# febrianrachmadi/dep-gan-im

Hardware: AMD Instinct MI355X
Metric: 2D slices/sec (G+2D+GP train step), 256x256x1 fp32 (higher is better)
Workload: dtype f32; 1 GPU; DEP-GAN-IM twoCritics canonical train step (critic-Y2 + critic-DEM + G update, WGAN-GP), batch 32 per GPU, 256x256x1; per_gpu_batch=32, global_batch=32, parallelism=dp1

## Files before the change

### dep_gan_im_amd/csrc/common.h

```cpp
#pragma once
#include <hip/hip_runtime.h>
#include <stdint.h>
#include <stddef.h>

typedef float f32x2 __attribute__((ext_vector_type(2)));
typedef float f32x4 __attribute__((ext_vector_type(4)));
typedef float f32x16 __attribute__((ext_vector_type(16)));

struct TView {
  float* p;
  long sB, sY, sX;
};

static inline TView make_view(float* p, int H, int W, int C) {
  TView v;
  v.p = p;
  v.sX = C;
  v.sY = (long)W * C;
  v.sB = (long)H * W * C;
  return v;
}
static inline TView make_view_slice(float* p, int H, int W, int Ctot, int c0) {
  TView v = make_view(p, H, W, Ctot);
  v.p = p + c0;
// ... 28 lines not shown
  TViewH v;
  v.p = nullptr;
  v.sB = v.sY = v.sX = 0;
  return v;
}

struct Epilogue {
  const float* bias;
  const float* scale;
  const float* shift;
  const float* film_mul;
  const float* film_add;
  int film_ld;
  TView out_pre;
  TView res;
  TView mask;
  int relu;
  int accumulate;
  TView pool;
  const float* head_w;
  const float* head_b;
  float* head_out;
  int head_tanh, head_skip_out;
};

struct ConvArgs {
  TView in;
  TView out;
  const float* w;
  int B, H, W, Cin, Cout;
  Epilogue ep;
  long wsT, wsI, wsO;
  int flip;
  int vec4;
  unsigned long long* dbg;
  int groups;
  int lgx, lgy;
  const float* w_group[4];
  long out_group_off[4];
  int cpt;
  long in_run_off[4];
};

struct WgradArgs {
  TView x;
  TView dy;
  float* part;
  int B, H, W, Cin, Cout;
  int nTiles, tilesPerChunk;
  float* colpart;
  int colB;
};

#ifdef __HIPCC__
static __device__ __forceinline__ float dg_vmax(float a, float b) {
  float o;
  asm("v_max_f32 %0, %1, %2" : "=v"(o) : "v"(a), "v"(b));
  return o;
}
#endif

#define DG_OK 0
#define DG_ERR_ARG 1
#define DG_ERR_HIP 2
#define DG_ERR_UNSUPPORTED 3

void dg_set_error(const char* fmt, ...);
// ... 85 lines not shown
  const float* src;
  float* dst;
  const float* kscale;
  int ntaps, srcI, srcO, io, transpose, flip;
  int NT, CK, nCC, Kdim, Ndim;
  int bf16;
  int tapg;
  int wino;
  unsigned total;
  unsigned per_nt;
  unsigned nt_stride;
  unsigned blk0, nblk;
};
int dg_pack_job(const ConvPlan& pl, const float* src, int srcI, int srcO, int io, int transpose, int flip,
                const float* kscale, float* dst, size_t nt_stride, PackJob* job);
unsigned dg_pack_layout(PackJob* jobs_host, int njobs);
int dg_pack_weights_batch(const PackJob* jobs_dev, int njobs, unsigned nblocks, hipStream_t st);

int dg_pack_weights(const ConvPlan& pl, const float* src, int srcI, int srcO, int io, int transpose, int flip,
                    const float* kscale, float* dst, hipStream_t st);

int dg_conv_igemm(const ConvPlan& pl, const ConvArgs& a, hipStream_t st);
int dg_conv_igemm_check(const ConvPlan& pl, const ConvArgs& a);
bool dg_conv_igemm_wp_supported(const ConvPlan& pl, const ConvArgs& a, bool force);
int dg_conv_igemm_wp(const ConvPlan& pl, const ConvArgs& a, hipStream_t st);
bool dg_conv_igemm_ws5_supported(const ConvPlan& pl, const ConvArgs& a, bool force);
int dg_conv_igemm_ws5(const ConvPlan& pl, const ConvArgs& a, hipStream_t st);
const char* dg_conv_igemm_ws5_name(const ConvPlan& pl);
int dg_conv_igemm_tile(const ConvPlan& pl, const ConvArgs& a, hipStream_t st);
bool dg_conv_igemm_head_supported(const ConvPlan& pl, const ConvArgs& a);
ConvPlan dg_plan_conv_wino(int Cin, int Cout);
bool dg_conv_wino_supported(const ConvPlan& pl, const ConvArgs& a);
const char* dg_conv_wino_name(const ConvArgs& a);
int dg_conv_wino(const ConvPlan& pl, const ConvArgs& a, hipStream_t st);
enum { DG_EPF_BIAS = 1, DG_EPF_AFFINE = 2, DG_EPF_FILM = 4, DG_EPF_RELU = 8, DG_EPF_PRE = 16, DG_EPF_RES = 32,
       DG_EPF_MASK = 64, DG_EPF_POOL = 128, DG_EPF_ACCUM = 256, DG_EPF_HEAD = 512, DG_EPF_ALL = 1023 };
unsigned dg_epilogue_flags(const Epilogue& e);
int dg_wino_epi_class(unsigned flags, int form);
void dg_set_epi_classes(int on);
int dg_get_epi_classes();
void dg_conv_igemm_name(const ConvPlan& pl, const ConvArgs& a, char* buf, size_t cap);
int dg_conv_direct(int KS, const ConvArgs& a, hipStream_t st);

int dg_wgrad(int KS, const WgradArgs& a, int* nchunks, hipStream_t st);
int dg_wgrad_finish(const float* part, int nchunks, int ntaps, int Cin, int Cout, const float* scale, float* out,
                    float* raw, int accumulate, int oi, const float* colpart, int colC, const float* colscale,
                    float* colout, float* colraw, hipStream_t st);
int dg_wgrad_finish_rows(const float* part, int nchunks, int ntaps, int Cin, int Cout, const float* scale, float* out,
                         float* raw, int accumulate, int oi, const float* colpart, int colrows, int colC,
                         const float* colscale, float* colout, float* colraw, hipStream_t st);

bool dg_wgrad_bf16_supported(int KS, int Cin, int Cout);
int dg_wgrad_bf16(int KS, const WgradArgs& a, int* nchunks, hipStream_t st);

int dg_wgrad_small(int KS, const WgradArgs& a, int* nchunks, hipStream_t st);

int dg_wgrad_plan(int KS, int B, int H, int W, int Cin, int Cout, int out[4]);
int dg_wgrad_small_plan(int KS, int B, int H, int W, int Cin, int Cout, int out[4]);
int dg_wgrad_bf16_plan(int KS, int B, int H, int W, int Cin, int Cout, int out[4]);

enum DgWgradKernel { DG_WG_F32 = 0, DG_WG_EDGE = 1, DG_WG_BF16 = 2, DG_WG_BF16S = 3, DG_WG_DECONV = 4 };
struct DgWgradChoice {
  int kernel, nchunks;
  size_t part_floats;
  int col_rows;
};
// ... 3 lines not shown
```

### dep_gan_im_amd/csrc/igemm_epilogue.inc

```
#ifndef EPI_PRE_SYNC
#define EPI_PRE_SYNC __syncthreads()
#define EPI_PRE_SYNC_DEFAULTED
#endif
  EPI_PRE_SYNC;
  constexpr int CP = NT + 4;
#ifdef EPI_ES_BASE
  float* es = EPI_ES_BASE;
#else
  float* es = smem + wv * (64 * CP);
#endif
  constexpr int NQ = (MF == 32) ? 4 : 1, CSTEP = (MF == 32) ? 8 : 4;
#if defined(EPI_STAGE)
  EPI_STAGE;
  (void)es;
#elif !defined(EPI_PHASED)
#pragma unroll
  for (int mt = 0; mt < MT; ++mt)
#pragma unroll
    for (int g = 0; g < NQ; ++g) {
      f32x4 q4;
#pragma unroll
      for (int k = 0; k < 4; ++k) q4[k] = acc[mt][4 * g + k];
      *reinterpret_cast<f32x4*>(es + (MF * mt + r) * CP + CSTEP * g + 4 * h) = q4;
    }
// ... 10 lines not shown
#ifndef EPI_OYW
  const int wvu = __builtin_amdgcn_readfirstlane(wv);
#endif
  const Epilogue& e = a.ep;
#ifdef EPI_CLASS
  typedef EPI_CLASS EpiC;
  constexpr bool EPI_CT = EpiC::fixed;
  const bool affine = EPI_CT ? EpiC::affine : (e.scale != nullptr), film = EPI_CT ? EpiC::film : (e.film_mul != nullptr),
             relu = EPI_CT ? EpiC::relu : (e.relu != 0), accum = EPI_CT ? false : (e.accumulate != 0);
  const bool has_bias = EPI_CT ? EpiC::bias : (e.bias != nullptr), has_pre = EPI_CT ? EpiC::pre : (e.out_pre.p != nullptr),
             has_res = EPI_CT ? EpiC::res : (e.res.p != nullptr), has_msk = EPI_CT ? EpiC::msk : (e.mask.p != nullptr),
             has_pool = EPI_CT ? EpiC::pool : (e.pool.p != nullptr);
#else
  const bool affine = e.scale != nullptr, film = e.film_mul != nullptr, relu = e.relu != 0, accum = e.accumulate != 0;
  const bool has_bias = e.bias != nullptr, has_pre = e.out_pre.p != nullptr, has_res = e.res.p != nullptr,
             has_msk = e.mask.p != nullptr, has_pool = e.pool.p != nullptr;
#endif
#ifdef EPI_OYW
  const int oyw = EPI_OYW;
#else
  const int oyw = ty0 + 4 * wvu;
#endif
#ifdef EPI_HEAD
  float hkeep_out = 0.f;
#endif
#ifdef EPI_FULL
  const bool full = EPI_FULL;
#else
  const bool full = (ty0 + 16 <= a.H) && (tx0 + 16 <= a.W);
#endif
  if (co < a.Cout) {
    f32x4 bias4 = {0.f, 0.f, 0.f, 0.f}, sc4 = {1.f, 1.f, 1.f, 1.f}, sh4 = {0.f, 0.f, 0.f, 0.f};
    f32x4 fm4 = {1.f, 1.f, 1.f, 1.f}, fa4 = {0.f, 0.f, 0.f, 0.f};
    if (has_bias) bias4 = *reinterpret_cast<const f32x4*>(e.bias + co);
    if (affine) {
      sc4 = *reinterpret_cast<const f32x4*>(e.scale + co);
      sh4 = *reinterpret_cast<const f32x4*>(e.shift + co);
    }
#pragma unroll
    for (int k = 0; k < 4; ++k) sh4[k] = fmaf(bias4[k], sc4[k], sh4[k]);
    if (film) {
      fm4 = *reinterpret_cast<const f32x4*>(e.film_mul + (long)b * e.film_ld + co);
      fa4 = *reinterpret_cast<const f32x4*>(e.film_add + (long)b * e.film_ld + co);
    }
    auto mk = [&](const float* p) {
      const unsigned long long u = (unsigned long long)p;
      const unsigned lo = __builtin_amdgcn_readfirstlane((unsigned)u), hi = __builtin_amdgcn_readfirstlane((unsigned)(u >> 32));
      return __builtin_amdgcn_make_buffer_rsrc((void*)(((unsigned long long)hi << 32) | lo), 0, 0x7FFFFFFF, 0x00020000);
    };
    const int lo_out = 4 * (pl0 * (int)a.out.sX + co);
    const int lo_pre = has_pre ? 4 * (pl0 * (int)e.out_pre.sX + co) : 0;
    const int lo_res = has_res ? 4 * (pl0 * (int)e.res.sX + co) : 0;
    const int lo_msk = has_msk ? 4 * (pl0 * (int)e.mask.sX + co) : 0;
    const __amdgpu_buffer_rsrc_t r_out = mk(a.out.p + out_goff + view_off(a.out, b, oyw, tx0));
    const __amdgpu_buffer_rsrc_t r_pre = mk(has_pre ? e.out_pre.p + view_off(e.out_pre, b, oyw, tx0) : a.out.p);
    const __amdgpu_buffer_rsrc_t r_res = mk(has_res ? e.res.p + view_off(e.res, b, oyw, tx0) : a.out.p);
    const __amdgpu_buffer_rsrc_t r_msk = mk(has_msk ? e.mask.p + view_off(e.mask, b, oyw, tx0) : a.out.p);
    const __amdgpu_buffer_rsrc_t r_pool =
        mk(has_pool ? e.pool.p + view_off(e.pool, b, oyw >> 1, tx0 >> 1) : a.out.p);
    const int lo_pool = has_pool ? 4 * ((pl0 >> 1) * (int)e.pool.sX + co) : 0;
    const int sY_pool = 4 * (int)e.pool.sY, sX_pool = 4 * (int)e.pool.sX;
    f32x4 vrow = {0.f, 0.f, 0.f, 0.f};
#ifdef EPI_HEAD
#ifdef EPI_CLASS
    const bool has_head = EPI_HEAD && (EPI_CT ? EpiC::head : (e.head_out != nullptr));
#else
    const bool has_head = EPI_HEAD && e.head_out != nullptr;
#endif
    f32x4 hw4 = {0.f, 0.f, 0.f, 0.f};
    if (has_head) hw4 = *reinterpret_cast<const f32x4*>(e.head_w + co);
    const bool skip_out = has_head && e.head_skip_out != 0;
#else
    constexpr bool has_head = false, skip_out = false;
#endif
    typedef int i32x4 __attribute__((ext_vector_type(4)));
    auto ld = [&](const __amdgpu_buffer_rsrc_t& r, int voff, int soff) {
      const i32x4 t = __builtin_amdgcn_raw_buffer_load_b128(r, voff, soff, 0);
      return __builtin_bit_cast(f32x4, t);
    };
    auto st = [&](const __amdgpu_buffer_rsrc_t& r, int voff, int soff, f32x4 v) {
      __builtin_amdgcn_raw_buffer_store_b128(__builtin_bit_cast(i32x4, v), r, voff, soff, 0);
    };
    const int sY_out = 4 * (int)a.out.sY, sX_out = 4 * (int)a.out.sX;
    const int sY_pre = 4 * (int)e.out_pre.sY, sX_pre = 4 * (int)e.out_pre.sX;
    const int sY_res = 4 * (int)e.res.sY, sX_res = 4 * (int)e.res.sX;
    const int sY_msk = 4 * (int)e.mask.sY, sX_msk = 4 * (int)e.mask.sX;
#ifdef EPI_STAGE_LATE
    EPI_STAGE_LATE;
#endif
#pragma unroll
    for (int p = 0; p < NPASS; ++p) {
      constexpr int RP = 16 / PPP;
      const int py = (p & 1) + 2 * (p / (2 * RP)), px0 = ((p >> 1) % RP) * PPP;
      const bool ok = full || (oyw + py < a.H && tx0 + px0 + pl0 < a.W);
#if defined(EPI_FETCH)
      f32x4 v;
      EPI_FETCH(v, py, (px0 + pl0));
#elif defined(EPI_PHASED)
      static_assert(MF == 32, "phased epilogue: 32-pixel tiles");
      if (p % (NPASS / MT) == 0) {
        const int mtp = p / (NPASS / MT);
#pragma unroll
        for (int g = 0; g < NQ; ++g) {
          f32x4 q4;
#pragma unroll
          for (int k = 0; k < 4; ++k) q4[k] = acc[mtp][4 * g + k];
          *reinterpret_cast<f32x4*>(es + r * CP + CSTEP * g + 4 * h) = q4;
        }
      }
      f32x4 v = *reinterpret_cast<const f32x4*>(es + ((py & 1) * 16 + px0 + pl0) * CP + c4);
#else
      f32x4 v = *reinterpret_cast<const f32x4*>(es + (py * 16 + px0 + pl0) * CP + c4);
#endif
#pragma unroll
      for (int k = 0; k < 4; ++k) v[k] = fmaf(v[k], sc4[k], sh4[k]);
      if (has_pre) {
        if (ok) st(r_pre, lo_pre, py * sY_pre + px0 * sX_pre, v);
      }
      if (film) {
#pragma unroll
        for (int k = 0; k < 4; ++k) v[k] = film_preact(v[k], fm4[k], fa4[k]);
      }
      if (relu) {
#pragma unroll
        for (int k = 0; k < 4; ++k) v[k] = dg_vmax(v[k], 0.f);
      }
      if (has_res) {
        f32x4 rr = {0.f, 0.f, 0.f, 0.f};
        if (ok) rr = ld(r_res, lo_res, py * sY_res + px0 * sX_res);
#pragma unroll
        for (int k = 0; k < 4; ++k) v[k] += rr[k];
      }
      if (has_msk) {
        f32x4 mm = {1.f, 1.f, 1.f, 1.f};
        if (ok) mm = ld(r_msk, lo_msk, py * sY_msk + px0 * sX_msk);
#pragma unroll
        for (int k = 0; k < 4; ++k) v[k] = (mm[k] > 0.f) ? v[k] : 0.f;
      }
      const int so = py * sY_out + px0 * sX_out;
      if (accum) {
        f32x4 old = {0.f, 0.f, 0.f, 0.f};
        if (ok) old = ld(r_out, lo_out, so);
#pragma unroll
        for (int k = 0; k < 4; ++k) v[k] += old[k];
      }
      if (ok && !skip_out) st(r_out, lo_out, so, v);
#ifdef EPI_HEAD
      if (has_head) {
        static_assert(!EPI_HEAD || (NT == 32 && NPASS == 8), "fused head: 32-channel tiles, eight passes");
        float d = v[0] * hw4[0];
        d = fmaf(v[1], hw4[1], d);
        d = fmaf(v[2], hw4[2], d);
        d = fmaf(v[3], hw4[3], d);
#define EPI_DPP(x, ctrl) \
  __builtin_bit_cast(float, __builtin_amdgcn_update_dpp(0, __builtin_bit_cast(int, (x)), (ctrl), 0xF, 0xF, false))
        d += EPI_DPP(d, 0xB1);
        d += EPI_DPP(d, 0x4E);
        d += EPI_DPP(d, 0x141);
#undef EPI_DPP
        hkeep_out = ((lane & 7) == p) ? d : hkeep_out;
      }
#endif
      if (has_pool) {
        if ((py & 1) == 0) {
          vrow = v;
        } else {
          f32x4 m;
#pragma unroll
          for (int k = 0; k < 4; ++k) {
            const float t = dg_vmax(vrow[k], v[k]);
            m[k] = dg_vmax(t, __shfl_xor(t, LPP, 64));
          }
          if (ok && (pl0 & 1) == 0) st(r_pool, lo_pool, (py >> 1) * sY_pool + (px0 >> 1) * sX_pool, m);
        }
      }
    }
  }
#ifdef EPI_HEAD
  if (EPI_HEAD && a.ep.head_out != nullptr && n0 < a.Cout) {
    const int ph = lane & 7, plh = lane >> 3;
    const int pyh = (ph & 1) + 2 * (ph >> 2), pxh = ((ph >> 1) & 1) * 8 + plh;
    const int yh = oyw + pyh, xh = tx0 + pxh;
    if (yh < a.H && xh < a.W) {
      const float t = hkeep_out + a.ep.head_b[0];
      a.ep.head_out[((long)b * a.H + yh) * a.W + xh] = a.ep.head_tanh ? tanhf(t) : t;
    }
  }
#endif
#ifdef EPI_PRE_SYNC_DEFAULTED
#undef EPI_PRE_SYNC
#undef EPI_PRE_SYNC_DEFAULTED
#endif
```

### dep_gan_im_amd/csrc/igemm_wino.hip

```cpp
#include <stdlib.h>

#include <type_traits>

#include "common.h"
#include "epilogue.h"

namespace {

constexpr int WN_CK = 8;
constexpr int WN_TW = 18;
constexpr int WN_CP = 36;
constexpr int WN_XV = WN_CK / 4;

template <int MT>
struct WnCfg {
  static constexpr int TH = 8 * MT;
  static constexpr int NTILE = 32 * MT;
  static constexpr int PIXT = (TH + 2) * WN_TW;
  static constexpr int XTOT = PIXT * WN_XV;
  static constexpr int NXP = (XTOT + 255) / 256;
  static constexpr int RAW = NXP * 256 * 4;
  static_assert(XTOT % 4 == 0 && WN_TW % 2 == 0, "rslot permutes inside aligned groups of four slots: halo and padding stay apart");
  static constexpr int ZPLANE = NTILE * WN_CP + 32;
  static constexpr int Z = 8 * ZPLANE;
// ... 57 lines not shown
  const unsigned nNTall = (unsigned)a.lgy, nPix = (unsigned)a.lgx;
  const int nCC = a.Cin / WN_CK;

  constexpr int SENT = (int)0x80000000;
  int xvo[NXP], xyx[NXP];
#pragma unroll
  for (int i = 0; i < NXP; ++i) {
    const int q = tid + i * 256;
    const int lq = rslot_inv(q);
    const int pix = lq >> 1, part = lq & 1;
    const int ly = pix / WN_TW, lx = pix - ly * WN_TW;
    xvo[i] = (q < WN_XTOT) ? 4 * (ly * (int)a.in.sY + lx * (int)a.in.sX + part * 4) : SENT;
    xyx[i] = (ly << 8) | lx;
  }
  int tA[MT][4], tB[MT][4];
  float tS[MT];
#pragma unroll
  for (int i = 0; i < MT; ++i) {
    const int cg = h, aa = wv, T = 32 * i + r;
    const int tyi = T >> 3, txi = T & 7;
    const int rA = (aa == 0) ? 0 : (aa == 2 ? 2 : 1), rB = (aa == 3) ? 3 : (aa == 2 ? 1 : 2);
#pragma unroll
    for (int j = 0; j < 4; ++j) {
      tA[i][j] = 16 * rslot((2 * tyi + rA) * WN_TW + 2 * txi + j, cg);
      tB[i][j] = 16 * rslot((2 * tyi + rB) * WN_TW + 2 * txi + j, cg);
    }
    tS[i] = (aa == 1) ? 1.f : -1.f;
  }
  const int wbase = __builtin_amdgcn_readfirstlane(wv * 256);
  const int wvo = 4 * ((4 * wv * 32 + r) * WN_CK + 4 * h);

  unsigned id = blockIdx.x;
  do {
    int t, ntile;
    if ((nPix & 7u) == 0) {
      const unsigned x = id & 7u, sl = id >> 3;
      ntile = (int)(sl % nNTall);
      t = (int)(x * (nPix >> 3) + sl / nNTall);
    } else {
      t = (int)(id % nPix);
      ntile = (int)(id / nPix);
    }
    const int tx0 = (t % tilesX) * 16;
    t /= tilesX;
    const int ty0 = (t % tilesY) * C::TH;
    const int b = t / tilesY;
    const long out_goff = 0;
    const int n0 = ntile * NT;
    const float* const xorg = a.in.p + ((long)b * a.in.sB + (long)(ty0 - 1) * (int)a.in.sY + (long)(tx0 - 1) * (int)a.in.sX);
    const unsigned long long xu = (unsigned long long)xorg;
    const unsigned xlo = __builtin_amdgcn_readfirstlane((unsigned)xu), xhi = __builtin_amdgcn_readfirstlane((unsigned)(xu >> 32));
    const __amdgpu_buffer_rsrc_t rx =
        __builtin_amdgcn_make_buffer_rsrc((void*)(((unsigned long long)xhi << 32) | xlo), 0, 0x7FFFFFFF, 0x00020000);
    int xvi[NXP];
#pragma unroll
    for (int i = 0; i < NXP; ++i) {
      const int iy = ty0 + (xyx[i] >> 8) - 1, ix = tx0 + (xyx[i] & 255) - 1;
      xvi[i] = ((unsigned)iy < (unsigned)a.H && (unsigned)ix < (unsigned)a.W) ? xvo[i] : SENT;
    }
    int xso = GATH ? 4 * (int)a.in_run_off[0] : 0;
    int grun = 0, gleft = GATH ? a.cpt : 0;
    auto next_chunk = [&]() {
      if constexpr (GATH) {
        if (--gleft == 0) {
          ++grun;
          gleft = a.cpt;
          xso = 4 * (int)a.in_run_off[grun];
        } else {
          xso += 4 * WN_CK;
        }
      } else {
        xso += 4 * WN_CK;
      }
    };
    auto stage_dma = [&](auto buf_tag) {
      constexpr int BUF = decltype(buf_tag)::value;
      float* xs = smem + BUF * WN_RAW + wbase;
#pragma unroll
      for (int i = 0; i < NXP; ++i) {
// ... 82 lines not shown
        if (rt_last) wn_wait_vm<0>();
        else wn_wait_vm<NXI>();
      } else {
        wn_wait_vm<LAST ? 0 : NXI>();
      }
      asm volatile("" : "+v"(bq[0]), "+v"(bq[1]), "+v"(bq[2]), "+v"(bq[3])::"memory");
#pragma unroll
      for (int f = 0; f < 4; ++f) {
        __builtin_amdgcn_sched_barrier(0);
#pragma unroll
        for (int j = 0; j < 4; ++j)
#pragma unroll
          for (int mt = 0; mt < MT; ++mt)
            if (!(ABL & 4)) {
              if (FIRST && j == 0) {
                const acc_t zero = {0.f, 0.f, 0.f, 0.f, 0.f, 0.f, 0.f, 0.f, 0.f, 0.f, 0.f, 0.f, 0.f, 0.f, 0.f, 0.f};
                acc[f][mt] = __builtin_amdgcn_mfma_f32_32x32x2f32(bq[f][j], vr[mt][f][j >> 1][j & 1], zero, 0, 0, 0);
              } else {
                acc[f][mt] = __builtin_amdgcn_mfma_f32_32x32x2f32(bq[f][j], vr[mt][f][j >> 1][j & 1], acc[f][mt], 0, 0, 0);
              }
            } else {
              if (FIRST && j == 0) acc[f][mt] = acc_t{};
              acc[f][mt][j] += bq[f][j] * vr[mt][f][j >> 1][j & 1];
            }
        __builtin_amdgcn_sched_barrier(0);
      }
    };
    {
      const std::true_type yes;
      const std::false_type no;
      const WnSlot<1> last;
      const WnSlot<0> more;
      const WnSlot<-1> rt;
      rt_last = nCC == 1;
      chunk(yes, WnSlot<0>{}, rt);
      if (nCC > 1) {
#pragma unroll 1
        for (int k = (nCC - 2) >> 1; k > 0; --k) {
          chunk(no, WnSlot<1>{}, more);
          chunk(no, WnSlot<0>{}, more);
        }
        if (nCC & 1) chunk(no, WnSlot<1>{}, more);
        rt_slot = (nCC - 1) & 1;
        chunk(no, rt, last);
      }
    }

    if (ABL & 1) {
      float sacc = 0.f;
#pragma unroll
      for (int f = 0; f < 4; ++f)
#pragma unroll
        for (int mt = 0; mt < MT; ++mt)
#pragma unroll
          for (int j = 0; j < 16; ++j) sacc += acc[f][mt][j];
      if (sacc == 12345.678f) a.out.p[tid] = sacc;
      __syncthreads();
      continue;
    }
    auto zstage = [&]() {
      __syncthreads();
      float* zw = smem + (2 * wv) * WN_ZPLANE + r * WN_CP + 4 * h;
#pragma unroll
      for (int mt = 0; mt < MT; ++mt)
#pragma unroll
        for (int g = 0; g < 4; ++g) {
          f32x4 z0, z1;
#pragma unroll
          for (int k = 0; k < 4; ++k) {
            const float m0 = acc[0][mt][4 * g + k], m1 = acc[1][mt][4 * g + k], m2 = acc[2][mt][4 * g + k],
                        m3 = acc[3][mt][4 * g + k];
            z0[k] = (m0 + m1) + m2;
            z1[k] = (m1 - m2) - m3;
          }
          *reinterpret_cast<f32x4*>(zw + mt * (32 * WN_CP) + 8 * g) = z0;
          *reinterpret_cast<f32x4*>(zw + WN_ZPLANE + mt * (32 * WN_CP) + 8 * g) = z1;
        }
      __syncthreads();
    };
#define EPI_PRE_SYNC
#define EPI_STAGE
#define EPI_STAGE_LATE zstage()
#define EPI_NPASS (4 * MT)
#define EPI_OYW (ty0 + 2 * MT * __builtin_amdgcn_readfirstlane(wv))
#define EPI_FULL ((ty0 + C::TH <= a.H) && (tx0 + 16 <= a.W))
#define EPI_FETCH(v, py, px)                                                                                         \
  {                                                                                                                  \
    const float* zb = smem + ((px)&1) * WN_ZPLANE +                                                                  \
                      ((MT * __builtin_amdgcn_readfirstlane(wv) + ((py) >> 1)) * 8 + ((px) >> 1)) * WN_CP + c4;       \
    const f32x4 za = *reinterpret_cast<const f32x4*>(zb + (((py)&1) ? 2 : 0) * WN_ZPLANE);                           \
    const f32x4 zb1 = *reinterpret_cast<const f32x4*>(zb + (((py)&1) ? 4 : 2) * WN_ZPLANE);                          \
    const f32x4 zc = *reinterpret_cast<const f32x4*>(zb + (((py)&1) ? 6 : 4) * WN_ZPLANE);                           \
    _Pragma("unroll") for (int k_ = 0; k_ < 4; ++k_) v[k_] = ((py)&1) ? (za[k_] - zb1[k_]) - zc[k_] : (za[k_] + zb1[k_]) + zc[k_]; \
  }
#define EPI_HEAD HEAD
#define EPI_CLASS WnEpi<EC>
#include "igemm_epilogue.inc"
#undef EPI_CLASS
#undef EPI_HEAD
#undef EPI_FETCH
#undef EPI_FULL
#undef EPI_OYW
#undef EPI_NPASS
#undef EPI_STAGE_LATE
#undef EPI_STAGE
#undef EPI_PRE_SYNC
    if (PERS) __syncthreads();
  } while (PERS && (id += gridDim.x) < nPix * nNTall);
}

template <int MT, bool PERS, int EC>
__global__ __launch_bounds__(256, WnCfg<MT>::WGS_PER_CU) void wino_conv_kernel(const ConvArgs a) {
  wino_body<MT, PERS, false, false, 0, EC>(a);
}
template <bool PERS, int EC>
__global__ __launch_bounds__(256, 2) void wino_conv_head_kernel(const ConvArgs a) {
  wino_body<2, PERS, true, false, 0, EC>(a);
}
template <int MT, bool PERS>
__global__ __launch_bounds__(256, WnCfg<MT>::WGS_PER_CU) void wino_conv_gathered_kernel(const ConvArgs a) {
  wino_body<MT, PERS, false, true>(a);
}
#ifdef DEPGAN_WINO_ABLATIONS
template <int MT, int ABL>
__global__ __launch_bounds__(256, WnCfg<MT>::WGS_PER_CU) void wino_conv_abl_kernel(const ConvArgs a) {
  wino_body<MT, true, false, false, ABL>(a);
}
#endif

struct WnKern {
  const void* fn;
  const char* name;
};
// ... 45 lines not shown
  return 0;
}

bool dg_conv_wino_supported(const ConvPlan& pl, const ConvArgs& a) {
  if (!dg_plan_wino(pl)) return false;
  if (a.Cin != pl.Cin || (a.Cin % WN_CK) || (a.Cout % 32) || a.groups > 1 || a.dbg || ((a.H | a.W) & 1)) return false;
  if (a.cpt > 0 && ((a.Cin % (a.cpt * WN_CK)) != 0 || a.Cin / (a.cpt * WN_CK) > 4)) return false;
  long run = 0;
  for (int t = 0; a.cpt > 0 && t < a.Cin / (a.cpt * WN_CK); ++t) {
    if (a.in_run_off[t] < 0) return false;
    run = a.in_run_off[t] > run ? a.in_run_off[t] : run;
  }
  constexpr long lim = 1L << 29;
  if (a.in.sY < 0 || a.in.sX < 0 || a.in.sY >= lim || a.in.sX >= lim || run >= lim) return false;
  if ((WnCfg<2>::TH + 2) * a.in.sY + WN_TW * a.in.sX + a.Cin + run >= lim) return false;
  return true;
}

static int wino_mt(const ConvArgs& a) {
  static int forced = -1;
  if (forced < 0) {
    const char* e = getenv("DEPGAN_WINO_MT");
    forced = e ? atoi(e) : 0;
  }
  if (a.ep.head_out) return 2;
  if (forced == 1 || forced == 2) return forced;
  return 1;
}

template <int MT>
static void wino_geometry(ConvArgs& a, long* total, long* G, bool* pers) {
  a.lgx = cdiv(a.W, 16) * cdiv(a.H, WnCfg<MT>::TH) * a.B;
  a.lgy = a.Cout / 32;
  *total = (long)a.lgx * a.lgy;
  const long cap = (long)WnCfg<MT>::WGS_PER_CU * dg_cu_count();
  *pers = *total > cap;
  *G = *pers ? cap : *total;
}

static const WnKern* wino_pick(const ConvArgs& a, int mt, bool pers) {
  const int form = a.ep.head_out ? 1 : (a.cpt > 0 ? 3 : (mt == 2 ? 2 : 0));
  const int ec = dg_wino_epi_class(dg_epilogue_flags(a.ep), form);
  if (form == 1) return &kWnHead[ec ? 1 : 0][pers];
  if (form == 3) return &kWnGath[mt - 1][pers];
  if (form == 2) return &kWn16[pers];
  return &kWn8[ec][pers];
}

const char* dg_conv_wino_name(const ConvArgs& a_in) {
  ConvArgs a = a_in;
  long total, G;
  bool pers;
  const int mt = wino_mt(a);
  if (mt == 2) wino_geometry<2>(a, &total, &G, &pers); else wino_geometry<1>(a, &total, &G, &pers);
  return wino_pick(a, mt, pers)->name;
}

template <int MT>
static int wino_launch(ConvArgs a, hipStream_t st) {
  long total, G;
  bool pers;
  wino_geometry<MT>(a, &total, &G, &pers);
  constexpr size_t LDS = WnCfg<MT>::LDS;
  static DgOncePerDevice once;
  if (once.need()) {
    const WnKern* const own = (MT == 2) ? &kWn16[0] : &kWn8[0][0];
    const int nown = (MT == 2) ? 2 : 2 * WN_HEAD_CLASS;
    for (int i = 0; i < nown; ++i)
      HIPCHECK(hipFuncSetAttribute(own[i].fn, hipFuncAttributeMaxDynamicSharedMemorySize, (int)LDS));
    for (int i = 0; i < 2; ++i)
      HIPCHECK(hipFuncSetAttribute(kWnGath[MT - 1][i].fn, hipFuncAttributeMaxDynamicSharedMemorySize, (int)LDS));
    for (int i = 0; MT == 2 && i < 4; ++i)
      HIPCHECK(hipFuncSetAttribute(kWnHead[i >> 1][i & 1].fn, hipFuncAttributeMaxDynamicSharedMemorySize, (int)LDS));
  }
#ifdef DEPGAN_WINO_ABLATIONS
  if (const char* e = getenv("DEPGAN_WINO_ABL")) {
    const int abl = atoi(e);
    if (abl && pers && !a.ep.head_out && a.cpt <= 0) {
#define WN_ABL_CASE(N)                                                                                              \
  case N:                                                                                                           \
    HIPCHECK(hipFuncSetAttribute(reinterpret_cast<const void*>(&wino_conv_abl_kernel<MT, N>),                       \
                                 hipFuncAttributeMaxDynamicSharedMemorySize, (int)LDS));                            \
    hipLaunchKernelGGL((wino_conv_abl_kernel<MT, N>), dim3((unsigned)G), dim3(256), LDS, st, a);                    \
    break;
      switch (abl) {
        WN_ABL_CASE(1) WN_ABL_CASE(2) WN_ABL_CASE(3) WN_ABL_CASE(4) WN_ABL_CASE(8) WN_ABL_CASE(10) WN_ABL_CASE(11)
        default: dg_set_error("DEPGAN_WINO_ABL=%d not instantiated", abl); return DG_ERR_ARG;
      }
// ... 25 lines not shown
```

### dep_gan_im_amd/csrc/op_entries.hip

```cpp
#include "model.h"

#include <math.h>
#include <stdlib.h>
#include <stdio.h>
#include <string.h>

int op_pack_jobs(PackJob* jobs, int n, hipStream_t st) {
  const unsigned nb = dg_pack_layout(jobs, n);
  DevTmp jd(st);
  DGCHECK(jd.alloc(n * sizeof(PackJob)));
  hipError_t e = hipMemcpyAsync(jd.p, jobs, n * sizeof(PackJob), hipMemcpyHostToDevice, st);
  if (e != hipSuccess) { dg_set_error("op_pack_jobs: upload failed: %s", hipGetErrorString(e)); return DG_ERR_HIP; }
  return dg_pack_weights_batch(jd.as<PackJob>(), n, nb, st);
}

static int op_alloc(DevTmp* t, size_t floats, const char* who) {
  if (t->alloc((floats ? floats : 1) * sizeof(float)) != DG_OK) {
    dg_set_error("%s: out of device memory (%zu floats)", who, floats);
    return DG_ERR_HIP;
  }
  return DG_OK;
}

template <typename XV>
// ... 253 lines not shown
int depgan_get_epilogue_classes(void) { return dg_get_epi_classes(); }
int depgan_wino_epilogue_class(unsigned flags, int form) {
  if ((flags & ~(unsigned)DG_EPF_ALL) || form < 0 || form > 3) {
    dg_set_error("wino_epilogue_class: flags 0x%x outside DEPGAN_EPF_ALL or form %d outside 0 ... 3", flags, form);
    return -1;
  }
  return dg_wino_epi_class(flags, form);
}
int depgan_op_conv3x3_wino_kernel_name(unsigned flags, int B, int H, int W, int Cin, int Cout, char* buf, int cap) {
  if ((flags & ~(unsigned)DG_EPF_ALL) || B < 1 || H < 1 || W < 1 || Cin < 1 || Cout < 1 || !buf || cap < 1) {
    dg_set_error("op_conv3x3_wino_kernel_name: null or non-positive argument, or flags outside DEPGAN_EPF_ALL");
    return DG_ERR_ARG;
  }
  static float present;
  const TView pv = make_view(&present, H, W, Cout);
  ConvArgs a = conv_args(make_view(&present, H, W, Cin), pv, B, H, W, Cin, Cout);
  Epilogue& e = a.ep;
  if (flags & DG_EPF_BIAS) e.bias = &present;
  if (flags & DG_EPF_AFFINE) e.scale = e.shift = &present;
  if (flags & DG_EPF_FILM) { e.film_mul = e.film_add = &present; e.film_ld = Cout; }
  e.relu = (flags & DG_EPF_RELU) ? 1 : 0;
  if (flags & DG_EPF_PRE) e.out_pre = pv;
  if (flags & DG_EPF_RES) e.res = pv;
  if (flags & DG_EPF_MASK) e.mask = pv;
  if (flags & DG_EPF_POOL) e.pool = pv;
  e.accumulate = (flags & DG_EPF_ACCUM) ? 1 : 0;
  if (flags & DG_EPF_HEAD) { e.head_w = e.head_b = &present; e.head_out = &present; }
  const ConvPlan pl = dg_plan_conv_wino(Cin, Cout);
  if (!dg_plan_wino(pl) || !dg_conv_wino_supported(pl, a)) {
    dg_set_error("op_conv3x3_wino_kernel_name: the Winograd kernel does not cover this shape");
    return DG_ERR_UNSUPPORTED;
  }
  snprintf(buf, (size_t)cap, "%s", dg_conv_wino_name(a));
  return DG_OK;
}

int depgan_op_deconv2x2_igemm(int form, const float* in, long isB, long isY, long isX, const float* w_hwoi,
                              const float* bias, const float* scale, const float* shift, float* out, long osB, long osY,
                              long osX, const float* mask, long msB, long msY, long msX, int B, int H, int W, int Cin,
                              int Cout, int relu, int path, void* stream) {
  if (op_view_bad_batched(in, isB, isY, isX) || op_view_bad_batched(out, osB, osY, osX) || !w_hwoi || B < 1 || H < 1 || W < 1 || Cin < 1 ||
      Cout < 1 || (mask && op_view_bad_batched(mask, msB, msY, msX))) {
    dg_set_error("op_deconv2x2_igemm: null or non-positive argument");
    return DG_ERR_ARG;
  }
  if (form < 0 || form > 2 || !scale != !shift || (path != 1 && path != 3 && path != 8)) {
    dg_set_error("op_deconv2x2_igemm: form must be 0, 1 or 2, path 1, 3 or 8, scale and shift come as a pair");
    return DG_ERR_ARG;
  }
  if (form == 0 ? mask != nullptr : (bias || scale || relu)) {
    dg_set_error("op_deconv2x2_igemm: the forward takes bias / scale / shift / relu, the backward-data forms a mask");
    return DG_ERR_ARG;
  }
  if (path == 8) { dg_set_error("op_deconv2x2_igemm: the Winograd kernel has no 1x1 form"); return DG_ERR_UNSUPPORTED; }
  auto plan = [&](int ci, int co) { return path == 3 ? dg_plan_conv_bf16(1, ci, co) : dg_plan_conv(1, ci, co); };
  auto covered = [&](const ConvPlan& p) { return dg_plan_mfma(p) && (path == 3) == dg_plan_bf16(p); };
  hipStream_t st = (hipStream_t)stream;
  ConvArgs a = conv_args(null_view(), null_view(), B, H, W, 0, 0);
  DevTmp wt(st);
  if (form == 0) {
    const ConvPlan pf = plan(Cin, Cout);
    if (!covered(pf)) { dg_set_error("op_deconv2x2_igemm: no MFMA plan for %d -> %d on path %d", Cin, Cout, path); return DG_ERR_UNSUPPORTED; }
    const TView o = op_view(out, osB, osY, osX);
    a.in = op_view(in, isB, isY, isX);
    a.Cin = Cin; a.Cout = Cout;
    a.ep.bias = bias; a.ep.scale = scale; a.ep.shift = shift; a.ep.relu = relu;
// ... 709 lines not shown
```

### include/depgan.h

```cpp
#ifndef DEPGAN_H
#define DEPGAN_H
#include <stddef.h>
#ifdef __cplusplus
extern "C" {
#endif

typedef struct depgan_ctx depgan_ctx;

#define DEPGAN_ABI_VERSION 3
int depgan_abi_version(void);
size_t depgan_config_size(void);
const char* depgan_source_hash(void);

typedef struct depgan_config {
  int struct_size;
  int batch;
  int height;
  int width;
  int nicg;
  int first_fm;
  float im_thresh;
  float delta;
  float lrD, lrG;
  float beta1, beta2, adam_eps;
// ... 240 lines not shown
int depgan_op_maxpool(const float* in, float* out, int B, int Ho, int Wo, int C, void* hip_stream);
int depgan_op_deconv2x2(const float* in, const float* w_hwoi, const float* bias, const float* scale,
                        const float* shift, float* out, int B, int H, int W, int Cin, int Cout, int relu,
                        void* hip_stream);

int depgan_op_deconv2x2_wgrad(const float* in, const float* dout, float* dw_hwoi, float* colsum, int B, int H, int W,
                              int Cin, int Cout, void* hip_stream);

int depgan_op_conv2d_fused(const float* in, long isB, long isY, long isX, const float* w_hwio, const float* bias,
                           const float* scale, const float* shift, const float* film_mul, const float* film_add,
                           int film_ld, float* out, long osB, long osY, long osX, float* out_pre, long psB, long psY,
                           long psX, const float* res, long rsB, long rsY, long rsX, const float* mask, long msB,
                           long msY, long msX, float* pool, long qsB, long qsY, long qsX, const float* head_w,
                           const float* head_b, float* head_out, int head_tanh, int head_skip_out, int B, int H, int W,
                           int Cin, int Cout, int KS, int relu, int accumulate, int path, int bwd, void* hip_stream);
int depgan_op_conv3x3_wino_gathered(const float* in, long isB, long isY, long isX, const long* run_off, int runs,
                                    const float* w_hwio, const float* bias, float* out, long osB, long osY, long osX,
                                    int B, int H, int W, int Cin, int Cout, void* hip_stream);
#define DEPGAN_EPF_BIAS 1
#define DEPGAN_EPF_AFFINE 2
#define DEPGAN_EPF_FILM 4
#define DEPGAN_EPF_RELU 8
#define DEPGAN_EPF_PRE 16
#define DEPGAN_EPF_RES 32
#define DEPGAN_EPF_MASK 64
#define DEPGAN_EPF_POOL 128
#define DEPGAN_EPF_ACCUM 256
#define DEPGAN_EPF_HEAD 512
#define DEPGAN_EPF_ALL 1023
int depgan_set_epilogue_classes(int on);
int depgan_get_epilogue_classes(void);
int depgan_wino_epilogue_class(unsigned flags, int form);
int depgan_op_conv3x3_wino_kernel_name(unsigned flags, int B, int H, int W, int Cin, int Cout, char* buf, int cap);
int depgan_op_deconv2x2_igemm(int form, const float* in, long isB, long isY, long isX, const float* w_hwoi,
                              const float* bias, const float* scale, const float* shift, float* out, long osB, long osY,
                              long osX, const float* mask, long msB, long msY, long msX, int B, int H, int W, int Cin,
                              int Cout, int relu, int path, void* hip_stream);
int depgan_op_conv2d_wgrad_ex(const float* x, long xsB, long xsY, long xsX, const float* dy, long dsB, long dsY,
                              long dsX, const float* scale, float* dw, float* raw, int accumulate, int oi, int colB,
                              const float* colscale, float* colout, float* colraw, int B, int H, int W, int Cin,
                              int Cout, int KS, int bf16, void* hip_stream);
int depgan_debug_wgrad_plan(int kernel, int KS, int B, int H, int W, int Cin, int Cout, int out[4]);
int depgan_debug_wgrad_choice(int KS, int B, int H, int W, int Cin, int Cout, int bf16_pipe, int x_bf16, long out[4]);

int depgan_op_bn_moments(const float* x, long sB, long sY, long sX, int B, int H, int W, int C, float* mean, float* var,
                         long scratch_floats, void* hip_stream);
int depgan_op_bn_backward(const float* dy, const float* raw, float* draw, long sB, long sY, long sX, int B, int H, int W,
                          int C, const float* gamma, const float* mean, const float* var, float eps, float invN,
                          float dyscale, float* dgamma, float* dbeta, long scratch_floats, void* hip_stream);
int depgan_op_affine_act(const float* in, float* out, float* out_pre, const float* res, long sB, long sY, long sX,
                         const float* s, const float* t, const float* film_mul, const float* film_add, int film_ld,
                         int relu, int B, int H, int W, int C, unsigned drop_seed, float drop_rate, void* hip_stream);
int depgan_op_softmax_ce4(const float* logits, const float* onehot, float* probs, float* dz, float* loss_sum, long P,
                          void* hip_stream);
int depgan_op_softmax_ce(const float* logits, const float* onehot, const unsigned char* codes, float* probs, float* dz,
                         float* loss_sum, long P, int C, void* hip_stream);
int depgan_op_softmax_ce_census(const float* logits, const float* onehot, const unsigned char* codes, float* probs,
                                float* dz, float* loss_sum, long long* census_host, long P, int C, void* hip_stream);
int depgan_op_softmax_ce_weighted(const float* logits, const float* onehot, const unsigned char* codes,
                                  const float* w_host, int n, int ignore_code, float* probs, float* dz, float* loss_sum,
                                  long long* census_host, long long* counts_host, long P, int C, void* hip_stream);
int depgan_op_softmax_ce_focal(const float* logits, const float* onehot, const unsigned char* codes, const float* w_host,
                               int n, int ignore_code, float gamma, float label_smoothing, float* probs, float* dz,
                               float* loss_sum, long long* census_host, long long* counts_host, long P, int C,
                               void* hip_stream);
int depgan_op_label_counts(const float* onehot, const unsigned char* codes, long P, int C, int ignore_code,
// ... 74 lines not shown
```

Measured before the change: 710.3 slices/s.

## Trim Winograd conv kernel scalar/vector overhead with shift-based tile decode and packed math

The persistent Winograd conv kernel now decodes work-item indices with host-precomputed log2 shifts and masks when the tile counts are powers of two, replacing integer division and modulo. The output transform and the epilogue affine now use packed two-wide float math, and the per-channel constant loads plus the LDS fetch addresses are rebuilt around a precomputed per-lane base pointer. For tiles with no boundary, a compile-time specialised epilogue path drops the per-store bounds checks and adds a store guard. These changes target ALU and address overhead in the kernel, at the cost of more macro complexity and a new debug entry point.

```diff
diff --git a/dep_gan_im_amd/csrc/common.h b/dep_gan_im_amd/csrc/common.h
--- a/dep_gan_im_amd/csrc/common.h
+++ b/dep_gan_im_amd/csrc/common.h
@@ -84,7 +84,10 @@
   Epilogue ep;
   long wsT, wsI, wsO;
   int flip;
-  int vec4;
+  union {
+    int vec4;
+    int wn_dec;
+  };
   unsigned long long* dbg;
   int groups;
   int lgx, lgy;
@@ -236,6 +239,9 @@
 ConvPlan dg_plan_conv_wino(int Cin, int Cout);
 bool dg_conv_wino_supported(const ConvPlan& pl, const ConvArgs& a);
 const char* dg_conv_wino_name(const ConvArgs& a);
+constexpr int DG_WN_DEC_NONE = 0x80;
+constexpr int DG_WN_DEC_NOXCD = (int)0x80000000u;
+void dg_conv_wino_item_plan(const ConvArgs& a, int out[4]);
 int dg_conv_wino(const ConvPlan& pl, const ConvArgs& a, hipStream_t st);
 enum { DG_EPF_BIAS = 1, DG_EPF_AFFINE = 2, DG_EPF_FILM = 4, DG_EPF_RELU = 8, DG_EPF_PRE = 16, DG_EPF_RES = 32,
        DG_EPF_MASK = 64, DG_EPF_POOL = 128, DG_EPF_ACCUM = 256, DG_EPF_HEAD = 512, DG_EPF_ALL = 1023 };
diff --git a/dep_gan_im_amd/csrc/igemm_epilogue.inc b/dep_gan_im_amd/csrc/igemm_epilogue.inc
--- a/dep_gan_im_amd/csrc/igemm_epilogue.inc
+++ b/dep_gan_im_amd/csrc/igemm_epilogue.inc
@@ -66,16 +66,20 @@
   if (co < a.Cout) {
     f32x4 bias4 = {0.f, 0.f, 0.f, 0.f}, sc4 = {1.f, 1.f, 1.f, 1.f}, sh4 = {0.f, 0.f, 0.f, 0.f};
     f32x4 fm4 = {1.f, 1.f, 1.f, 1.f}, fa4 = {0.f, 0.f, 0.f, 0.f};
-    if (has_bias) bias4 = *reinterpret_cast<const f32x4*>(e.bias + co);
+#ifndef EPI_LDC
+#define EPI_LDC(p) (*reinterpret_cast<const f32x4*>((p) + co))
+#define EPI_LDC_DEFAULTED
+#endif
+    if (has_bias) bias4 = EPI_LDC(e.bias);
     if (affine) {
-      sc4 = *reinterpret_cast<const f32x4*>(e.scale + co);
-      sh4 = *reinterpret_cast<const f32x4*>(e.shift + co);
+      sc4 = EPI_LDC(e.scale);
+      sh4 = EPI_LDC(e.shift);
     }
 #pragma unroll
     for (int k = 0; k < 4; ++k) sh4[k] = fmaf(bias4[k], sc4[k], sh4[k]);
     if (film) {
-      fm4 = *reinterpret_cast<const f32x4*>(e.film_mul + (long)b * e.film_ld + co);
-      fa4 = *reinterpret_cast<const f32x4*>(e.film_add + (long)b * e.film_ld + co);
+      fm4 = EPI_LDC(e.film_mul + (long)b * e.film_ld);
+      fa4 = EPI_LDC(e.film_add + (long)b * e.film_ld);
     }
     auto mk = [&](const float* p) {
       const unsigned long long u = (unsigned long long)p;
@@ -102,7 +106,7 @@
     const bool has_head = EPI_HEAD && e.head_out != nullptr;
 #endif
     f32x4 hw4 = {0.f, 0.f, 0.f, 0.f};
-    if (has_head) hw4 = *reinterpret_cast<const f32x4*>(e.head_w + co);
+    if (has_head) hw4 = EPI_LDC(e.head_w);
     const bool skip_out = has_head && e.head_skip_out != 0;
 #else
     constexpr bool has_head = false, skip_out = false;
@@ -122,12 +126,33 @@
 #ifdef EPI_STAGE_LATE
     EPI_STAGE_LATE;
 #endif
+#ifdef EPI_SPLIT_FULL
+    auto epi_passes = [&](auto full_tag) {
+    constexpr bool FULLC = decltype(full_tag)::value;
+    constexpr bool SPLIT = EPI_SPLIT_FULL;
+#define EPI_ST_GUARD                                 \
+  do {                                               \
+    if (FULLC) {                                     \
+      asm volatile("s_nop 3" ::: "memory");          \
+      __builtin_amdgcn_sched_barrier(0);             \
+    }                                                \
+  } while (0)
+#else
+#define EPI_ST_GUARD
+#endif
 #pragma unroll
     for (int p = 0; p < NPASS; ++p) {
       constexpr int RP = 16 / PPP;
       const int py = (p & 1) + 2 * (p / (2 * RP)), px0 = ((p >> 1) % RP) * PPP;
+#ifdef EPI_SPLIT_FULL
+      const bool ok = FULLC || (!SPLIT && full) || (oyw + py < a.H && tx0 + px0 + pl0 < a.W);
+#else
       const bool ok = full || (oyw + py < a.H && tx0 + px0 + pl0 < a.W);
-#if defined(EPI_FETCH)
+#endif
+#if defined(EPI_FETCH0)
+      f32x4 v;
+      EPI_FETCH0(v, py, px0);
+#elif defined(EPI_FETCH)
       f32x4 v;
       EPI_FETCH(v, py, (px0 + pl0));
 #elif defined(EPI_PHASED)
@@ -146,10 +171,21 @@
 #else
       f32x4 v = *reinterpret_cast<const f32x4*>(es + (py * 16 + px0 + pl0) * CP + c4);
 #endif
+#ifdef EPI_PACKED
+      {
+        const f32x2 lo_ = __builtin_elementwise_fma(f32x2{v[0], v[1]}, f32x2{sc4[0], sc4[1]}, f32x2{sh4[0], sh4[1]});
+        const f32x2 hi_ = __builtin_elementwise_fma(f32x2{v[2], v[3]}, f32x2{sc4[2], sc4[3]}, f32x2{sh4[2], sh4[3]});
+        v = f32x4{lo_[0], lo_[1], hi_[0], hi_[1]};
+      }
+#else
 #pragma unroll
       for (int k = 0; k < 4; ++k) v[k] = fmaf(v[k], sc4[k], sh4[k]);
+#endif
       if (has_pre) {
-        if (ok) st(r_pre, lo_pre, py * sY_pre + px0 * sX_pre, v);
+        if (ok) {
+          st(r_pre, lo_pre, py * sY_pre + px0 * sX_pre, v);
+          EPI_ST_GUARD;
+        }
       }
       if (film) {
 #pragma unroll
@@ -178,7 +214,10 @@
 #pragma unroll
         for (int k = 0; k < 4; ++k) v[k] += old[k];
       }
-      if (ok && !skip_out) st(r_out, lo_out, so, v);
+      if (ok && !skip_out) {
+        st(r_out, lo_out, so, v);
+        EPI_ST_GUARD;
+      }
 #ifdef EPI_HEAD
       if (has_head) {
         static_assert(!EPI_HEAD || (NT == 32 && NPASS == 8), "fused head: 32-channel tiles, eight passes");
@@ -205,11 +244,24 @@
             const float t = dg_vmax(vrow[k], v[k]);
             m[k] = dg_vmax(t, __shfl_xor(t, LPP, 64));
           }
-          if (ok && (pl0 & 1) == 0) st(r_pool, lo_pool, (py >> 1) * sY_pool + (px0 >> 1) * sX_pool, m);
+          if (ok && (pl0 & 1) == 0) {
+            st(r_pool, lo_pool, (py >> 1) * sY_pool + (px0 >> 1) * sX_pool, m);
+            EPI_ST_GUARD;
+          }
         }
       }
     }
+#ifdef EPI_SPLIT_FULL
+    };
+    if (EPI_SPLIT_FULL && full) epi_passes(std::true_type{});
+    else epi_passes(std::false_type{});
+#endif
+#undef EPI_ST_GUARD
   }
+#ifdef EPI_LDC_DEFAULTED
+#undef EPI_LDC
+#undef EPI_LDC_DEFAULTED
+#endif
 #ifdef EPI_HEAD
   if (EPI_HEAD && a.ep.head_out != nullptr && n0 < a.Cout) {
     const int ph = lane & 7, plh = lane >> 3;
diff --git a/dep_gan_im_amd/csrc/igemm_wino.hip b/dep_gan_im_amd/csrc/igemm_wino.hip
--- a/dep_gan_im_amd/csrc/igemm_wino.hip
+++ b/dep_gan_im_amd/csrc/igemm_wino.hip
@@ -113,19 +113,38 @@
 
   unsigned id = blockIdx.x;
   do {
+    int dec = a.wn_dec;
+    asm volatile("" : "+s"(dec));
     int t, ntile;
-    if ((nPix & 7u) == 0) {
+    if ((dec & DG_WN_DEC_NOXCD) == 0) {
       const unsigned x = id & 7u, sl = id >> 3;
-      ntile = (int)(sl % nNTall);
-      t = (int)(x * (nPix >> 3) + sl / nNTall);
+      unsigned q;
+      if ((dec & DG_WN_DEC_NONE) == 0) {
+        const int lnt = dec & 31;
+        ntile = (int)(sl & ((1u << lnt) - 1));
+        q = sl >> lnt;
+      } else {
+        ntile = (int)(sl % nNTall);
+        q = sl / nNTall;
+      }
+      t = (int)(x * (nPix >> 3) + q);
     } else {
       t = (int)(id % nPix);
       ntile = (int)(id / nPix);
     }
-    const int tx0 = (t % tilesX) * 16;
-    t /= tilesX;
-    const int ty0 = (t % tilesY) * C::TH;
-    const int b = t / tilesY;
+    int tx0, ty0, b;
+    if ((dec & (DG_WN_DEC_NONE * 0x010100)) == 0) {
+      const int ltx = (dec >> 8) & 31, lty = (dec >> 16) & 31;
+      tx0 = (t & ((1 << ltx) - 1)) * 16;
+      t >>= ltx;
+      ty0 = (t & ((1 << lty) - 1)) * C::TH;
+      b = t >> lty;
+    } else {
+      tx0 = (t % tilesX) * 16;
+      t /= tilesX;
+      ty0 = (t % tilesY) * C::TH;
+      b = t / tilesY;
+    }
     const long out_goff = 0;
     const int n0 = ntile * NT;
     const float* const xorg = a.in.p + ((long)b * a.in.sB + (long)(ty0 - 1) * (int)a.in.sY + (long)(tx0 - 1) * (int)a.in.sX);
@@ -274,16 +293,18 @@
       const WnSlot<1> last;
       const WnSlot<0> more;
       const WnSlot<-1> rt;
-      rt_last = nCC == 1;
+      int ncc = nCC;
+      asm volatile("" : "+s"(ncc));
+      rt_last = ncc == 1;
       chunk(yes, WnSlot<0>{}, rt);
-      if (nCC > 1) {
+      if (ncc > 1) {
 #pragma unroll 1
-        for (int k = (nCC - 2) >> 1; k > 0; --k) {
+        for (int k = (ncc - 2) >> 1; k > 0; --k) {
           chunk(no, WnSlot<1>{}, more);
           chunk(no, WnSlot<0>{}, more);
         }
-        if (nCC & 1) chunk(no, WnSlot<1>{}, more);
-        rt_slot = (nCC - 1) & 1;
+        if (ncc & 1) chunk(no, WnSlot<1>{}, more);
+        rt_slot = (ncc - 1) & 1;
         chunk(no, rt, last);
       }
     }
@@ -307,40 +328,56 @@
       for (int mt = 0; mt < MT; ++mt)
 #pragma unroll
         for (int g = 0; g < 4; ++g) {
-          f32x4 z0, z1;
-#pragma unroll
-          for (int k = 0; k < 4; ++k) {
-            const float m0 = acc[0][mt][4 * g + k], m1 = acc[1][mt][4 * g + k], m2 = acc[2][mt][4 * g + k],
-                        m3 = acc[3][mt][4 * g + k];
+          f32x2 z0[2], z1[2];
+#pragma unroll
+          for (int k = 0; k < 2; ++k) {
+            const int j = 4 * g + 2 * k;
+            const f32x2 m0 = {acc[0][mt][j], acc[0][mt][j + 1]}, m1 = {acc[1][mt][j], acc[1][mt][j + 1]},
+                        m2 = {acc[2][mt][j], acc[2][mt][j + 1]}, m3 = {acc[3][mt][j], acc[3][mt][j + 1]};
             z0[k] = (m0 + m1) + m2;
             z1[k] = (m1 - m2) - m3;
           }
-          *reinterpret_cast<f32x4*>(zw + mt * (32 * WN_CP) + 8 * g) = z0;
-          *reinterpret_cast<f32x4*>(zw + WN_ZPLANE + mt * (32 * WN_CP) + 8 * g) = z1;
+          *reinterpret_cast<f32x4*>(zw + mt * (32 * WN_CP) + 8 * g) = f32x4{z0[0][0], z0[0][1], z0[1][0], z0[1][1]};
+          *reinterpret_cast<f32x4*>(zw + WN_ZPLANE + mt * (32 * WN_CP) + 8 * g) = f32x4{z1[0][0], z1[0][1], z1[1][0], z1[1][1]};
         }
       __syncthreads();
     };
 #define EPI_PRE_SYNC
 #define EPI_STAGE
-#define EPI_STAGE_LATE zstage()
+    int zt_ = tid;
+    asm volatile("" : "+v"(zt_));
+    static_assert(4 * (6 * WN_ZPLANE + ((2 * MT - 1) * 8 + 4) * WN_CP) + 16 <= 65536, "immediate offsets of the fetches");
+#define EPI_STAGE_LATE                                                                                                \
+  zstage();                                                                                                          \
+  const char* const zl = reinterpret_cast<const char*>(                                                              \
+      smem + ((zt_ >> 3) & 1) * WN_ZPLANE + (MT * 8 * (zt_ >> 6) + ((zt_ >> 4) & 3)) * WN_CP + (zt_ & 7) * 4)
 #define EPI_NPASS (4 * MT)
 #define EPI_OYW (ty0 + 2 * MT * __builtin_amdgcn_readfirstlane(wv))
 #define EPI_FULL ((ty0 + C::TH <= a.H) && (tx0 + 16 <= a.W))
-#define EPI_FETCH(v, py, px)                                                                                         \
+#define EPI_FETCH0(v, py, px0)                                                                                       \
   {                                                                                                                  \
-    const float* zb = smem + ((px)&1) * WN_ZPLANE +                                                                  \
-                      ((MT * __builtin_amdgcn_readfirstlane(wv) + ((py) >> 1)) * 8 + ((px) >> 1)) * WN_CP + c4;       \
-    const f32x4 za = *reinterpret_cast<const f32x4*>(zb + (((py)&1) ? 2 : 0) * WN_ZPLANE);                           \
-    const f32x4 zb1 = *reinterpret_cast<const f32x4*>(zb + (((py)&1) ? 4 : 2) * WN_ZPLANE);                          \
-    const f32x4 zc = *reinterpret_cast<const f32x4*>(zb + (((py)&1) ? 6 : 4) * WN_ZPLANE);                           \
-    _Pragma("unroll") for (int k_ = 0; k_ < 4; ++k_) v[k_] = ((py)&1) ? (za[k_] - zb1[k_]) - zc[k_] : (za[k_] + zb1[k_]) + zc[k_]; \
-  }
+    const char* zb = zl + 4 * (((py) >> 1) * 8 + ((px0) >> 1)) * WN_CP;                                              \
+    const f32x4 za = *reinterpret_cast<const f32x4*>(zb + 4 * (((py)&1) ? 2 : 0) * WN_ZPLANE);                       \
+    const f32x4 zb1 = *reinterpret_cast<const f32x4*>(zb + 4 * (((py)&1) ? 4 : 2) * WN_ZPLANE);                      \
+    const f32x4 zc = *reinterpret_cast<const f32x4*>(zb + 4 * (((py)&1) ? 6 : 4) * WN_ZPLANE);                       \
+    const f32x2 a0_ = {za[0], za[1]}, a1_ = {za[2], za[3]}, b0_ = {zb1[0], zb1[1]}, b1_ = {zb1[2], zb1[3]},         \
+                c0_ = {zc[0], zc[1]}, c1_ = {zc[2], zc[3]};                                                          \
+    const f32x2 lo_ = ((py)&1) ? (a0_ - b0_) - c0_ : (a0_ + b0_) + c0_;                                              \
+    const f32x2 hi_ = ((py)&1) ? (a1_ - b1_) - c1_ : (a1_ + b1_) + c1_;                                              \
+    v = f32x4{lo_[0], lo_[1], hi_[0], hi_[1]};                                                                       \
+  }
+#define EPI_LDC(p) (*reinterpret_cast<const f32x4*>(reinterpret_cast<const char*>((p) + n0) + (unsigned)((zt_ & 7) << 4)))
+#define EPI_PACKED
+#define EPI_SPLIT_FULL WnEpi<EC>::fixed
 #define EPI_HEAD HEAD
 #define EPI_CLASS WnEpi<EC>
 #include "igemm_epilogue.inc"
 #undef EPI_CLASS
 #undef EPI_HEAD
-#undef EPI_FETCH
+#undef EPI_SPLIT_FULL
+#undef EPI_PACKED
+#undef EPI_LDC
+#undef EPI_FETCH0
 #undef EPI_FULL
 #undef EPI_OYW
 #undef EPI_NPASS
@@ -452,6 +489,13 @@
 static void wino_geometry(ConvArgs& a, long* total, long* G, bool* pers) {
   a.lgx = cdiv(a.W, 16) * cdiv(a.H, WnCfg<MT>::TH) * a.B;
   a.lgy = a.Cout / 32;
+  auto lg = [](int n) {
+    int l = 0;
+    while ((1 << l) < n) ++l;
+    return (1 << l) == n ? l : DG_WN_DEC_NONE;
+  };
+  a.wn_dec = lg(a.lgy) | (lg(cdiv(a.W, 16)) << 8) | (lg(cdiv(a.H, WnCfg<MT>::TH)) << 16) |
+             ((a.lgx & 7) ? DG_WN_DEC_NOXCD : 0);
   *total = (long)a.lgx * a.lgy;
   const long cap = (long)WnCfg<MT>::WGS_PER_CU * dg_cu_count();
   *pers = *total > cap;
@@ -474,6 +518,18 @@
   const int mt = wino_mt(a);
   if (mt == 2) wino_geometry<2>(a, &total, &G, &pers); else wino_geometry<1>(a, &total, &G, &pers);
   return wino_pick(a, mt, pers)->name;
+}
+
+void dg_conv_wino_item_plan(const ConvArgs& a_in, int out[4]) {
+  ConvArgs a = a_in;
+  long total, G;
+  bool pers;
+  if (wino_mt(a) == 2) wino_geometry<2>(a, &total, &G, &pers); else wino_geometry<1>(a, &total, &G, &pers);
+  for (int i = 0; i < 3; ++i) {
+    const int l = (a.wn_dec >> (8 * ((i + 1) % 3))) & 0xFF;
+    out[i] = l == DG_WN_DEC_NONE ? -1 : l;
+  }
+  out[3] = pers ? 1 : 0;
 }
 
 template <int MT>
diff --git a/dep_gan_im_amd/csrc/op_entries.hip b/dep_gan_im_amd/csrc/op_entries.hip
--- a/dep_gan_im_amd/csrc/op_entries.hip
+++ b/dep_gan_im_amd/csrc/op_entries.hip
@@ -309,6 +309,22 @@
     return DG_ERR_UNSUPPORTED;
   }
   snprintf(buf, (size_t)cap, "%s", dg_conv_wino_name(a));
+  return DG_OK;
+}
+int depgan_wino_item_plan(int B, int H, int W, int Cin, int Cout, int head, int out[4]) {
+  if (B < 1 || H < 1 || W < 1 || Cin < 1 || Cout < 1 || (head != 0 && head != 1) || !out) {
+    dg_set_error("wino_item_plan: null or non-positive argument, or head outside 0 / 1");
+    return DG_ERR_ARG;
+  }
+  static float present;
+  ConvArgs a = conv_args(make_view(&present, H, W, Cin), make_view(&present, H, W, Cout), B, H, W, Cin, Cout);
+  if (head) { a.ep.head_w = a.ep.head_b = &present; a.ep.head_out = &present; }
+  const ConvPlan pl = dg_plan_conv_wino(Cin, Cout);
+  if (!dg_plan_wino(pl) || !dg_conv_wino_supported(pl, a)) {
+    dg_set_error("wino_item_plan: the Winograd kernel does not cover this shape");
+    return DG_ERR_UNSUPPORTED;
+  }
+  dg_conv_wino_item_plan(a, out);
   return DG_OK;
 }
 
diff --git a/include/depgan.h b/include/depgan.h
--- a/include/depgan.h
+++ b/include/depgan.h
@@ -296,6 +296,7 @@
 int depgan_get_epilogue_classes(void);
 int depgan_wino_epilogue_class(unsigned flags, int form);
 int depgan_op_conv3x3_wino_kernel_name(unsigned flags, int B, int H, int W, int Cin, int Cout, char* buf, int cap);
+int depgan_wino_item_plan(int B, int H, int W, int Cin, int Cout, int head, int out[4]);
 int depgan_op_deconv2x2_igemm(int form, const float* in, long isB, long isY, long isX, const float* w_hwoi,
                               const float* bias, const float* scale, const float* shift, float* out, long osB, long osY,
                               long osX, const float* mask, long msB, long msY, long msX, int B, int H, int W, int Cin,
```

After: 713.6 slices/s (median of 6 runs). No clear change (+0.5%).
